# bliunlpr/Robust_e2e_gan

Measured on AMD Instinct MI355X. Metric: joint_train utterances/sec, higher is better.
Workload: dtype f32; 1 GPU; config4: joint_train.py full GAN+ASR step, B=32 per GPU, T=800, F=257->80, L=40, V=4233, enhancer 2xBLSTM-256, VGG+3xBLSTMP-512, loc-attention decoder 300, D basic ndf64, Adadelta; global_batch=32, per_rank_batch=32, parallelism=dp1, utterance_lengths=560..800 frames (mean 680 of T=800)

## Files before the change

robust_e2e_gan_amd/csrc/wino44.hip:

```cpp
#include <hip/hip_runtime.h>
#include "../../include/re2e.h"
#include "common.h"

namespace {

template <class T>
__device__ __forceinline__ void bt5(const T& d0, const T& d1, const T& d2, const T& d3, const T& d4, T (&r)[5]) {
  r[0] = 2.f * d0 - d1 - 2.f * d2 + d3;
  r[1] = -2.f * d1 - d2 + d3;
  r[2] = 2.f * d1 - 3.f * d2 + d3;
  r[3] = d3 - d1;
  r[4] = 2.f * d1 - d2 - 2.f * d3 + d4;
}
__device__ __forceinline__ void g4(float k0, float k1, float k2, float k3, float (&r)[5]) {
  r[0] = 0.5f * k0;
  r[1] = -0.5f * (k0 + k1 + k2 + k3);
  r[2] = (-k0 + k1 - k2 + k3) * (1.f / 6.f);
  r[3] = (k0 + 2.f * k1 + 4.f * k2 + 8.f * k3) * (1.f / 6.f);
  r[4] = k3;
}

__global__ __launch_bounds__(256) void w44_filter_kernel(const float* __restrict__ w, int Cout, int Cin, int dgrad, float* __restrict__ U) {
  const int Cp = dgrad ? Cout : Cin, Op = dgrad ? Cin : Cout;
  const long i = (long)blockIdx.x * 256 + threadIdx.x;
// ... 53 lines not shown
  float* vp = V + p * tile_stride + c4 * 4;
#pragma unroll
  for (int a = 0; a < 5; ++a) {
    f32x4 r[5];
    bt5(t[a][0], t[a][1], t[a][2], t[a][3], t[a][4], r);
#pragma unroll
    for (int b = 0; b < 5; ++b) *reinterpret_cast<f32x4*>(vp + (long)(a * 5 + b) * pos_stride) = r[b];
  }
}

__global__ __launch_bounds__(256) void w44_output_kernel(const float* __restrict__ M, long P, int Cout, int OH, int OW, int ty, int tx,
                                                         float* __restrict__ out) {
  const int o4n = Cout >> 2;
  const long i = (long)blockIdx.x * 256 + threadIdx.x;
  if (i >= P * o4n) return;
  const int o4 = (int)(i % o4n);
  const long p = i / o4n;
  const int x = (int)(p % tx), y = (int)((p / tx) % ty), n = (int)(p / ((long)tx * ty));
  const float* mp = M + p * Cout + o4 * 4;
  const long ps = P * Cout;
  f32x4 s[2][5];
#pragma unroll
  for (int b = 0; b < 5; ++b) {
    f32x4 m[5];
#pragma unroll
    for (int a = 0; a < 5; ++a) m[a] = *reinterpret_cast<const f32x4*>(mp + (long)(a * 5 + b) * ps);
    s[0][b] = m[0] + m[1] + m[2] + m[3];
    s[1][b] = m[1] - m[2] + 2.f * m[3] + m[4];
  }
#pragma unroll
  for (int a = 0; a < 2; ++a) {
    const int oy = 2 * y + a;
    if (oy >= OH) continue;
    const f32x4 y0 = s[a][0] + s[a][1] + s[a][2] + s[a][3];
    const f32x4 y1 = s[a][1] - s[a][2] + 2.f * s[a][3] + s[a][4];
    float* op = out + (((long)n * OH + oy) * OW + 2 * x) * Cout + o4 * 4;
    *reinterpret_cast<f32x4*>(op) = y0;
    if (2 * x + 1 < OW) *reinterpret_cast<f32x4*>(op + Cout) = y1;
  }
}

template <class T>
__device__ __forceinline__ void a5(const T& y0, const T& y1, T (&r)[5]) {
  r[0] = y0; r[1] = y0 + y1; r[2] = y0 - y1; r[3] = y0 + 2.f * y1; r[4] = y1;
}
__global__ __launch_bounds__(256) void w44_dout_kernel(const float* __restrict__ dy, int NI, int OH, int OW, int Cout, int ty, int tx, long P, long Ppad,
                                                       float* __restrict__ dM) {
  const int o4n = Cout >> 2;
  const long i = (long)blockIdx.x * 256 + threadIdx.x;
  if (i >= Ppad * o4n) return;
  const int o4 = (int)(i % o4n);
  const long p = i / o4n;
  const int x = (int)(p % tx), y = (int)((p / tx) % ty), n = p < P ? (int)(p / ((long)tx * ty)) : -1;
  const f32x4 zero = {0.f, 0.f, 0.f, 0.f};
  f32x4 g[2][2];
#pragma unroll
  for (int a = 0; a < 2; ++a)
#pragma unroll
    for (int b = 0; b < 2; ++b) {
      const int oy = 2 * y + a, ox = 2 * x + b;
      g[a][b] = (n >= 0 && oy < OH && ox < OW) ? *reinterpret_cast<const f32x4*>(dy + (((long)n * OH + oy) * OW + ox) * Cout + o4 * 4) : zero;
    }
  f32x4 t0[5], t1[5];
  a5(g[0][0], g[1][0], t0);
  a5(g[0][1], g[1][1], t1);
  float* mp = dM + p * Cout + o4 * 4;
  const long ps = Ppad * Cout;
#pragma unroll
  for (int a = 0; a < 5; ++a) {
    f32x4 r[5];
    a5(t0[a], t1[a], r);
#pragma unroll
    for (int b = 0; b < 5; ++b) *reinterpret_cast<f32x4*>(mp + (long)(a * 5 + b) * ps) = r[b];
  }
}

__global__ __launch_bounds__(256) void w44_wgrad_final_kernel(const float* __restrict__ slabs, int C, int Cout, int sub, float* __restrict__ gw, float beta) {
  const long i = (long)blockIdx.x * 256 + threadIdx.x;
  if (i >= (long)C * Cout) return;
  const int o = (int)(i % Cout), c = (int)(i / Cout);
  const long ss = (long)C * Cout;
  float u[5][5];
#pragma unroll
  for (int pos = 0; pos < 25; ++pos) {
    float v = 0.f;
    for (int z = 0; z < sub; ++z) v += slabs[((long)pos * sub + z) * ss + i];
    u[pos / 5][pos % 5] = v;
  }
  auto gt = [](float v0, float v1, float v2, float v3, float v4, float (&r)[4]) {
    const float s6 = 1.f / 6.f;
    r[0] = 0.5f * v0 - 0.5f * v1 - s6 * v2 + s6 * v3;
    r[1] = -0.5f * v1 + s6 * v2 + 2.f * s6 * v3;
    r[2] = -0.5f * v1 - s6 * v2 + 4.f * s6 * v3;
    r[3] = -0.5f * v1 + s6 * v2 + 8.f * s6 * v3 + v4;
  };
  float t[4][5];
#pragma unroll
  for (int y = 0; y < 5; ++y) {
    float r[4];
    gt(u[0][y], u[1][y], u[2][y], u[3][y], u[4][y], r);
#pragma unroll
    for (int a = 0; a < 4; ++a) t[a][y] = r[a];
  }
  float* wp = gw + ((long)o * C + c) * 16;
#pragma unroll
  for (int a = 0; a < 4; ++a) {
    float r[4];
    gt(t[a][0], t[a][1], t[a][2], t[a][3], t[a][4], r);
#pragma unroll
    for (int b = 0; b < 4; ++b) wp[a * 4 + b] = beta != 0.f ? wp[a * 4 + b] + r[b] : r[b];
  }
}

struct W44Plan { int OH, OW, ty, tx; long P; size_t u_off, v_off, m_off, total; };
W44Plan w44_plan(int NI, int H, int W, int C, int Cout, int pad) {
  W44Plan p;
  p.OH = H + 2 * pad - 3; p.OW = W + 2 * pad - 3;
  p.ty = (p.OH + 1) / 2; p.tx = (p.OW + 1) / 2;
  p.P = (long)NI * p.ty * p.tx;
  auto up = [](size_t b) { return (b + 255) & ~(size_t)255; };
  p.u_off = 0;
  p.v_off = up((size_t)25 * C * Cout * 4);
  p.m_off = p.v_off + up((size_t)p.P * 25 * C * 4);
  p.total = p.m_off + up((size_t)p.P * 25 * Cout * 4);
  return p;
}
}

WinoFit wino4x4_fit(int NI, int H, int W, int C, int Cout, int pad) {
  if (C % 16 || Cout % 4) return kWinoChannels;
  const W44Plan p = w44_plan(NI, H, W, C, Cout, pad);
  return p.P * 25 * C * 4 >= 0xFFFFFFF0L || (long)Cout * 25 * C * 4 >= 0xFFFFFFF0L || p.P >= 0x7fffffffL ? kWinoBytes : kWinoFits;
}

extern "C" size_t re2e_conv4x4_wino_workspace_bytes(int NI, int H, int W, int C, int Cout, int pad) {
  if (NI <= 0 || H <= 0 || W <= 0 || C <= 0 || Cout <= 0 || pad < 0 || H + 2 * pad < 4 || W + 2 * pad < 4) return 0;
  return w44_plan(NI, H, W, C, Cout, pad).total;
}

extern "C" int re2e_conv4x4_wino(const float* in, int NI, int H, int W, int C, const float* w, int Cout, int pad, int dgrad, float* out,
                                 void* workspace, size_t workspace_bytes, hipStream_t stream) {
  RE2E_CHECK_ARG(in && w && out && workspace, "null operand");
  RE2E_CHECK_ARG(NI > 0 && H > 0 && W > 0 && C > 0 && Cout > 0 && pad >= 0 && H + 2 * pad >= 4 && W + 2 * pad >= 4, "bad geometry");
  const WinoFit fit = wino4x4_fit(NI, H, W, C, Cout, pad);
  if (fit == kWinoChannels) { re2e_set_error("re2e_conv4x4_wino: C must be a multiple of 16 and Cout of 4 (got %d, %d)", C, Cout); return RE2E_EUNSUPPORTED; }
  const W44Plan p = w44_plan(NI, H, W, C, Cout, pad);
  RE2E_CHECK_ARG(workspace_bytes >= p.total, "workspace too small (re2e_conv4x4_wino_workspace_bytes)");
  RE2E_CHECK_ARG((reinterpret_cast<uintptr_t>(in) & 15) == 0 && (reinterpret_cast<uintptr_t>(out) & 15) == 0 &&
                 (reinterpret_cast<uintptr_t>(workspace) & 15) == 0, "in / out / workspace must be 16-byte aligned");
  if (fit != kWinoFits) {
    re2e_set_error("re2e_conv4x4_wino: transformed operand larger than 4 GiB");
    return RE2E_EUNSUPPORTED;
  }
  float* U = reinterpret_cast<float*>(static_cast<char*>(workspace) + p.u_off);
  float* V = reinterpret_cast<float*>(static_cast<char*>(workspace) + p.v_off);
  float* M = reinterpret_cast<float*>(static_cast<char*>(workspace) + p.m_off);
  hipLaunchKernelGGL(w44_filter_kernel, dim3((unsigned)cdiv((long)C * Cout, 256)), dim3(256), 0, stream, w, dgrad ? C : Cout, dgrad ? Cout : C, dgrad, U);
  hipLaunchKernelGGL(w44_input_kernel, dim3((unsigned)cdiv(p.P * (C / 4), 256)), dim3(256), 0, stream, in, NI, H, W, C, pad, p.ty, p.tx, V, 25L * C, (long)C, p.P);
  static const bool log_calls = getenv("RE2E_IGEMM_LOG") != nullptr;
  if (log_calls)
    fprintf(stderr, "[igemm] A=W44%s B=DenseK tile=256x128x16 vec=1 M=%ld N=%d K=%d splits=25\n", dgrad ? "D" : "F", (long)NI * p.OH * p.OW, Cout, 16 * C);
  const int rc = gemm_kslices((int)p.P, Cout, 25 * C, 25, V, 25L * C, U, 25L * C, M, stream, 1);
  if (rc != RE2E_OK) return rc;
  hipLaunchKernelGGL(w44_output_kernel, dim3((unsigned)cdiv(p.P * (Cout / 4), 256)), dim3(256), 0, stream, M, p.P, Cout, p.OH, p.OW, p.ty, p.tx, out);
  RE2E_LAUNCH_CHECK();
  return RE2E_OK;
}

namespace {
struct W44WgradPlan { int OH, OW, ty, tx, sub; long P, Ppad; size_t v_off, m_off, s_off, total; };
W44WgradPlan w44_wgrad_plan(int NI, int H, int W, int C, int Cout, int pad) {
  W44WgradPlan p;
  p.OH = H + 2 * pad - 3; p.OW = W + 2 * pad - 3;
  p.ty = (p.OH + 1) / 2; p.tx = (p.OW + 1) / 2;
  p.P = (long)NI * p.ty * p.tx;
  const long tiles = (long)cdiv(C, 128) * cdiv(Cout, 128) * 25;
  int sub = (int)((1024 + tiles - 1) / tiles);
  const long maxsub = p.P / (16 * 64);
  if (sub > maxsub) sub = (int)maxsub;
  if (sub < 1) sub = 1;
  p.sub = sub;
  const long q = 16L * sub;
  p.Ppad = (p.P + q - 1) / q * q;
  auto up = [](size_t b) { return (b + 255) & ~(size_t)255; };
  p.v_off = 0;
  p.m_off = up((size_t)25 * p.Ppad * C * 4);
  p.s_off = p.m_off + up((size_t)25 * p.Ppad * Cout * 4);
  p.total = p.s_off + up((size_t)25 * sub * C * Cout * 4);
  return p;
}
}

WinoFit wino4x4_wgrad_fit(int NI, int H, int W, int C, int Cout, int pad) {
  if (C % 4 || Cout % 4) return kWinoChannels;
  return 25 * w44_wgrad_plan(NI, H, W, C, Cout, pad).Ppad * (long)(C > Cout ? C : Cout) * 4 >= 0xFFFFFFF0L ? kWinoBytes : kWinoFits;
}

extern "C" size_t re2e_conv4x4_wino_wgrad_workspace_bytes(int NI, int H, int W, int C, int Cout, int pad) {
  if (NI <= 0 || H <= 0 || W <= 0 || C <= 0 || Cout <= 0 || pad < 0 || H + 2 * pad < 4 || W + 2 * pad < 4) return 0;
  return w44_wgrad_plan(NI, H, W, C, Cout, pad).total;
}

extern "C" int re2e_conv4x4_wino_wgrad(const float* in, int NI, int H, int W, int C, const float* dout, int Cout, int pad, float* gw, float beta,
                                       void* workspace, size_t workspace_bytes, hipStream_t stream) {
  RE2E_CHECK_ARG(in && dout && gw && workspace, "null operand");
  RE2E_CHECK_ARG(NI > 0 && H > 0 && W > 0 && C > 0 && Cout > 0 && pad >= 0 && H + 2 * pad >= 4 && W + 2 * pad >= 4, "bad geometry");
  RE2E_CHECK_ARG(beta == 0.f || beta == 1.f, "beta must be 0 or 1");
  const WinoFit fit = wino4x4_wgrad_fit(NI, H, W, C, Cout, pad);
  if (fit == kWinoChannels) { re2e_set_error("re2e_conv4x4_wino_wgrad: C and Cout must be multiples of 4 (got %d, %d)", C, Cout); return RE2E_EUNSUPPORTED; }
  const W44WgradPlan p = w44_wgrad_plan(NI, H, W, C, Cout, pad);
  RE2E_CHECK_ARG(workspace_bytes >= p.total, "workspace too small (re2e_conv4x4_wino_wgrad_workspace_bytes)");
  RE2E_CHECK_ARG((reinterpret_cast<uintptr_t>(in) & 15) == 0 && (reinterpret_cast<uintptr_t>(dout) & 15) == 0 &&
                 (reinterpret_cast<uintptr_t>(workspace) & 15) == 0, "in / dout / workspace must be 16-byte aligned");
  if (fit != kWinoFits) { re2e_set_error("re2e_conv4x4_wino_wgrad: transformed operand larger than 4 GiB"); return RE2E_EUNSUPPORTED; }
  float* V = reinterpret_cast<float*>(static_cast<char*>(workspace) + p.v_off);
  float* dM = reinterpret_cast<float*>(static_cast<char*>(workspace) + p.m_off);
  float* S = reinterpret_cast<float*>(static_cast<char*>(workspace) + p.s_off);
  hipLaunchKernelGGL(w44_input_kernel, dim3((unsigned)cdiv(p.Ppad * (C / 4), 256)), dim3(256), 0, stream, in, NI, H, W, C, pad, p.ty, p.tx, V, (long)C,
                     p.Ppad * C, p.Ppad);
  hipLaunchKernelGGL(w44_dout_kernel, dim3((unsigned)cdiv(p.Ppad * (Cout / 4), 256)), dim3(256), 0, stream, dout, NI, p.OH, p.OW, Cout, p.ty, p.tx, p.P,
                     p.Ppad, dM);
  static const bool log_calls = getenv("RE2E_IGEMM_LOG") != nullptr;
  if (log_calls)
    fprintf(stderr, "[igemm] A=W44W B=DenseM tile=128x128x16 vec=1 M=%d N=%d K=%ld splits=%d\n", 16 * C, Cout, (long)NI * p.OH * p.OW, 25 * p.sub);
  const int rc = gemm_kslices_tn(C, Cout, (int)(25 * p.Ppad), 25 * p.sub, V, (long)C, dM, (long)Cout, S, stream, 1);
  if (rc != RE2E_OK) return rc;
  hipLaunchKernelGGL(w44_wgrad_final_kernel, dim3((unsigned)cdiv((long)C * Cout, 256)), dim3(256), 0, stream, S, C, Cout, p.sub, gw, beta);
  RE2E_LAUNCH_CHECK();
  return RE2E_OK;
}
```

robust_e2e_gan_amd/csrc/igemm.hip:

```cpp
#include <stdlib.h>
#include <type_traits>

#include "common.h"

namespace {

template <int WM_, int WN_, int TM_, int TN_, int BK_>
struct Cfg {
  static constexpr int WM = WM_, WN = WN_, TM = TM_, TN = TN_, BK = BK_;
  static constexpr int BM = WM_ * TM_ * 32, BN = WN_ * TN_ * 32;
  static constexpr int THREADS = WM_ * WN_ * 64;
  static constexpr int LDK = BK_ + 4;
};

struct DenseK {
  static constexpr bool KMAJ = true;
  static constexpr const char* NAME = "DenseK";
  static constexpr bool IS_CONVK = false;
  const float* p; unsigned nbytes; long ld; int rows, K;
  struct Row { unsigned base; };
  struct Kst { int k; };
  __device__ void init_row(Row& r, int row) const { r.base = row < rows ? (unsigned)((long)row * ld * 4) : nbytes; }
  __device__ void init_k(Kst& s, int k) const { s.k = k; }
  __device__ void advance(Kst& s, int bk) const { s.k += bk; }
// ... 455 lines not shown
          outp[rb + colv[b]] = sg * mulp[rb + colv[b]];
        }
      }
    return;
  }
  if (ep.beta != 0.f) {
#pragma unroll
    for (int a = 0; a < CF::TM; ++a)
#pragma unroll
      for (int b = 0; b < CF::TN; ++b) {
        float old[16];
        long offs[16];
#pragma unroll
        for (int r = 0; r < 16; ++r) {
          const long rb = row_base(m0 + (wm * CF::TM + a) * 32 + (r & 3) + 8 * (r >> 2) + 4 * lh);
          offs[r] = (rb >= 0 && colv[b] < ep.N) ? rb + colv[b] : -1;
          old[r] = offs[r] >= 0 ? ep.C[offs[r]] : 0.f;
        }
#pragma unroll
        for (int r = 0; r < 16; ++r)
          if (offs[r] >= 0) ep.C[offs[r]] = apply_act(acc[a][b][r] + bv[b], ep.act) + old[r];
      }
    return;
  }
  if (ep.act == RE2E_ACT_TANH || ep.act == RE2E_ACT_SIGMOID) {
    const bool th = ep.act == RE2E_ACT_TANH;
#pragma unroll
    for (int a = 0; a < CF::TM; ++a)
#pragma unroll
      for (int r = 0; r < 16; ++r) {
        const long rb = row_base(m0 + (wm * CF::TM + a) * 32 + (r & 3) + 8 * (r >> 2) + 4 * lh);
        if (rb < 0) continue;
#pragma unroll
        for (int b = 0; b < CF::TN; ++b) {
          const float v = acc[a][b][r] + bv[b];
          if (colv[b] < ep.N) ep.C[rb + colv[b]] = th ? tanhf_(v) : sigmoidf_(v);
        }
      }
    return;
  }
  {
    const float slope = ep.act == RE2E_ACT_RELU ? 0.f : (ep.act == RE2E_ACT_LRELU ? 0.2f : 1.f);
    const bool relu = ep.act == RE2E_ACT_RELU;
#pragma unroll
    for (int a = 0; a < CF::TM; ++a)
#pragma unroll
      for (int r = 0; r < 16; ++r) {
        const long rb = row_base(m0 + (wm * CF::TM + a) * 32 + (r & 3) + 8 * (r >> 2) + 4 * lh);
        if (rb < 0) continue;
#pragma unroll
        for (int b = 0; b < CF::TN; ++b) {
          const float v = acc[a][b][r] + bv[b];
          if (colv[b] < ep.N) ep.C[rb + colv[b]] = v < 0.f ? (relu ? 0.f : slope * v) : v;
        }
      }
  }
}

__global__ void splitk_reduce_kernel(const float* ws, int nsplit, int M, int N, float* C, long ldc, float beta,
                                     int conv_perm, int Cin, int KHW, const float* bias, const float* bias2, int act) {
  long i = (long)blockIdx.x * blockDim.x + threadIdx.x;
  long tot = (long)M * N;
  if (i >= tot) return;
  float s = 0.f;
  for (int z = 0; z < nsplit; ++z) s += ws[(long)z * tot + i];
  int m = (int)(i / N), n = (int)(i % N);
  long off;
  if (conv_perm) { int ci = m % Cin; int tap = m / Cin; off = ((long)n * Cin + ci) * KHW + tap; }
  else off = (long)m * ldc + n;
  if (bias) s += bias[n];
  if (bias2) s += bias2[n];
  s = apply_act(s, act);
  if (beta != 0.f) s += C[off];
  C[off] = s;
}

__global__ __launch_bounds__(1024) void splitk_reduce_wide_kernel(const float* ws, int nsplit, int M, int N, float* C, long ldc,
                                                                  float beta, int conv_perm, int Cin, int KHW) {
  __shared__ float part[16][64];
  const int e = threadIdx.x & 63, sl = threadIdx.x >> 6;
  const long tot = (long)M * N;
  const long i = (long)blockIdx.x * 64 + e;
  float s = 0.f;
  if (i < tot)
    for (int z = sl; z < nsplit; z += 16) s += ws[(long)z * tot + i];
  part[sl][e] = s;
  __syncthreads();
  if (sl != 0 || i >= tot) return;
  s = 0.f;
#pragma unroll
  for (int q = 0; q < 16; ++q) s += part[q][e];
  int m = (int)(i / N), n = (int)(i % N);
  long off;
  if (conv_perm) { int ci = m % Cin; int tap = m / Cin; off = ((long)n * Cin + ci) * KHW + tap; }
  else off = (long)m * ldc + n;
  if (beta != 0.f) s += C[off];
  C[off] = s;
}

template <bool TB, bool VEC>
__global__ __launch_bounds__(512) void skinny_gemm_kernel(const float* __restrict__ A, long lda, const float* __restrict__ B, long ldb,
                                                          float* C, long ldc, int M, int N, int K, const float* __restrict__ bias,
                                                          const float* __restrict__ bias2, float beta) {
  __shared__ float red[8][32][33];
  const int tid = threadIdx.x, lane = tid & 63, wid = tid >> 6, lr = lane & 31, lh = lane >> 5;
  const int n0 = blockIdx.x * 32;
  const int kq = (K + 7) / 8;
  const int per = (kq + 7) / 8;
  const int q0 = wid * per, q1 = min(kq, q0 + per);
  const int row = lr, col = n0 + lr;
  const bool rok = row < M, cok = col < N;
  const float* ap = A + (long)(rok ? row : 0) * lda;
  f32x16 acc;
#pragma unroll
  for (int r = 0; r < 16; ++r) acc[r] = 0.f;
  for (int qb = q0; qb < q1; qb += 4) {
    float av[4][4], bv[4][4];
#pragma unroll
    for (int u = 0; u < 4; ++u) {
      const int k = 8 * (qb + u) + 4 * lh;
      const bool qok = qb + u < q1;
      if (VEC) {
        const bool kok = qok && k < K;
        const f32x4 zero = {0.f, 0.f, 0.f, 0.f};
        const f32x4 a4 = (kok && rok) ? *reinterpret_cast<const f32x4*>(ap + k) : zero;
        f32x4 b4 = zero;
        if (TB) { if (kok && cok) b4 = *reinterpret_cast<const f32x4*>(B + (long)col * ldb + k); }
#pragma unroll
        for (int j = 0; j < 4; ++j) {
          av[u][j] = a4[j];
          bv[u][j] = TB ? b4[j] : ((kok && cok) ? B[(long)(k + j) * ldb + col] : 0.f);
        }
      } else {
#pragma unroll
        for (int j = 0; j < 4; ++j) {
          const bool kok = qok && k + j < K;
          av[u][j] = (kok && rok) ? ap[k + j] : 0.f;
          bv[u][j] = (kok && cok) ? (TB ? B[(long)col * ldb + k + j] : B[(long)(k + j) * ldb + col]) : 0.f;
        }
      }
    }
#pragma unroll
    for (int u = 0; u < 4; ++u)
#pragma unroll
      for (int j = 0; j < 4; ++j) acc = __builtin_amdgcn_mfma_f32_32x32x2f32(av[u][j], bv[u][j], acc, 0, 0, 0);
  }
#pragma unroll
  for (int r = 0; r < 16; ++r) red[wid][(r & 3) + 8 * (r >> 2) + 4 * lh][lr] = acc[r];
  __syncthreads();
  for (int i = tid; i < 32 * 32; i += 512) {
    const int m = i >> 5, n = n0 + (i & 31);
    if (m < M && n < N) {
      float v = 0.f;
#pragma unroll
      for (int w = 0; w < 8; ++w) v += red[w][m][i & 31];
      if (bias) v += bias[n];
      if (bias2) v += bias2[n];
      float* c = C + (long)m * ldc + n;
      *c = (beta != 0.f ? *c : 0.f) + v;
    }
  }
}

__global__ __launch_bounds__(512) void skinny_gemm2_kernel(const float* __restrict__ A, long lda, int M, int K, const float* __restrict__ B1, long ldb1,
                                                           int N1, float* C1, long ldc1, const float* __restrict__ B2, long ldb2, int N2,
                                                           float* C2, long ldc2) {
  __shared__ float red[8][32][33];
  const int tid = threadIdx.x, lane = tid & 63, wid = tid >> 6, lr = lane & 31, lh = lane >> 5;
// ... 775 lines not shown
```

robust_e2e_gan_amd/csrc/wino_wgrad.hip:

```cpp
#include <hip/hip_runtime.h>
#include "../../include/re2e.h"
#include "common.h"

namespace {
typedef float f32x16 __attribute__((ext_vector_type(16)));
typedef float f32x2 __attribute__((ext_vector_type(2)));
constexpr unsigned WW_OOB = 0x80000000u;
constexpr int WW_CB = 64, WW_OB = 32;

struct WwArgs {
  const float* x; const float* dy; float* slabs;
  int NI, H, W, C, Cout;
  int px, py, npatch, nsplit, ncb, nblk;
  unsigned x_bytes, dy_bytes;
  const int* row_lim;
  int flat;
  int dbg;
};

template <int TXW>
__global__ __launch_bounds__(256, 2) void wino_wgrad_kernel(WwArgs p) {
  constexpr int TYH = 32 / TXW, PW = 2 * TXW, PH = 2 * TYH;
  constexpr int XW = PW + 2, XH = PH + 2, XPIX = XW * XH;
  constexpr int XIT = (XPIX * 16 + 255) / 256, DIT = PW * PH * 8 / 256;
// ... 37 lines not shown
  auto store_patch = [&]() {
#pragma unroll
    for (int it = 0; it < XIT; ++it) {
      const int item = it * 256 + tid;
      if (item < XPIX * 16) *reinterpret_cast<f32x4*>(xs + item * 4) = xr[it];
    }
#pragma unroll
    for (int it = 0; it < DIT; ++it) *reinterpret_cast<f32x4*>(ds + (it * 256 + tid) * 4) = dr[it];
  };

  const int rA = wid == 0 ? 0 : (wid == 2 ? 2 : 1), rB = wid == 3 ? 3 : (wid == 2 ? 1 : 2);
  const float sg = wid == 1 ? 1.f : -1.f;
  const float a0 = wid == 3 ? 0.f : 1.f, a1 = wid == 0 ? 0.f : (wid == 1 ? 1.f : -1.f);
  constexpr int HR = TYH / 2;
  const float* xA = xs + ((rA + 2 * HR * lh) * XW) * WW_CB + 2 * lr;
  const float* xB = xs + ((rB + 2 * HR * lh) * XW) * WW_CB + 2 * lr;
  const float* dB = ds + (2 * HR * lh * PW) * WW_OB + lr;

  f32x16 acc[4][2];
#pragma unroll
  for (int j = 0; j < 4; ++j)
#pragma unroll
    for (int ct = 0; ct < 2; ++ct)
#pragma unroll
      for (int r = 0; r < 16; ++r) acc[j][ct][r] = 0.f;

  for (int pi = pbeg; pi < pend; ++pi) {
    if (p.row_lim) {
      const int n = pi / (p.py * p.px), pyi = (pi - n * (p.py * p.px)) / p.px;
      if (pyi * PH >= p.row_lim[n]) continue;
    }
    load_patch(pi);
    store_patch();
    __syncthreads();
    f32x2 t[4], v[2][4];
    float m[2][4];
    auto prep = [&](const int s, f32x2 (&vv)[4], float (&mm)[4]) {
      const int tyl = s / TXW, txl = s % TXW;
#pragma unroll
      for (int j = 0; j < 4; ++j) {
        if (txl != 0 && j < 2) { t[j] = t[j + 2]; continue; }
        const f32x2 da = *reinterpret_cast<const f32x2*>(xA + ((2 * tyl) * XW + 2 * txl + j) * WW_CB);
        const f32x2 db = *reinterpret_cast<const f32x2*>(xB + ((2 * tyl) * XW + 2 * txl + j) * WW_CB);
        t[j] = da + sg * db;
      }
      vv[0] = t[0] - t[2]; vv[1] = t[1] + t[2]; vv[2] = t[2] - t[1]; vv[3] = t[1] - t[3];
      const float e00 = dB[((2 * tyl) * PW + 2 * txl) * WW_OB], e01 = dB[((2 * tyl) * PW + 2 * txl + 1) * WW_OB];
      const float e10 = dB[((2 * tyl + 1) * PW + 2 * txl) * WW_OB], e11 = dB[((2 * tyl + 1) * PW + 2 * txl + 1) * WW_OB];
      const float s0 = a0 * e00 + a1 * e10, s1 = a0 * e01 + a1 * e11;
      mm[0] = s0; mm[1] = s0 + s1; mm[2] = s0 - s1; mm[3] = -s1;
    };
    prep(0, v[0], m[0]);
#pragma unroll
    for (int s = 0; s < 16; ++s) {
      if (s + 1 < 16) prep(s + 1, v[(s + 1) & 1], m[(s + 1) & 1]);
#pragma unroll
      for (int j = 0; j < 4; ++j) {
        acc[j][0] = __builtin_amdgcn_mfma_f32_32x32x2f32(v[s & 1][j][0], m[s & 1][j], acc[j][0], 0, 0, 0);
        acc[j][1] = __builtin_amdgcn_mfma_f32_32x32x2f32(v[s & 1][j][1], m[s & 1][j], acc[j][1], 0, 0, 0);
      }
      if (s + 1 < 16) {
#pragma unroll
        for (int g = 0; g < 8; ++g) {
          __builtin_amdgcn_sched_group_barrier(0x008, 1, 0);
          __builtin_amdgcn_sched_group_barrier(0x100, 1, 0);
          __builtin_amdgcn_sched_group_barrier(0x002, 4, 0);
        }
      }
    }
    __syncthreads();
  }
  float* sl = p.slabs + ((long)split * 16 + 4 * wid) * p.C * p.Cout;
#pragma unroll
  for (int j = 0; j < 4; ++j)
#pragma unroll
    for (int ct = 0; ct < 2; ++ct)
#pragma unroll
      for (int r = 0; r < 16; ++r) {
        const int c = c0 + 2 * ((r & 3) + 8 * (r >> 2) + 4 * lh) + ct;
        sl[((long)j * p.C + c) * p.Cout + o0 + lr] = acc[j][ct][r];
      }
}

__global__ __launch_bounds__(1024) void wino_wgrad_reduce_kernel(const float* __restrict__ slabs, int nsplit, long tot, float* __restrict__ red) {
  __shared__ float part[16][64];
  const int e = threadIdx.x & 63, sl = threadIdx.x >> 6;
  const long i = (long)blockIdx.x * 64 + e;
  float s = 0.f;
  if (i < tot)
    for (int z = sl; z < nsplit; z += 16) s += slabs[(long)z * tot + i];
  part[sl][e] = s;
  __syncthreads();
  if (sl != 0 || i >= tot) return;
  s = 0.f;
#pragma unroll
  for (int q = 0; q < 16; ++q) s += part[q][e];
  red[i] = s;
}

__global__ __launch_bounds__(256) void wino_wgrad_final_kernel(const float* __restrict__ slabs, int nsplit, int C, int Cout, float* __restrict__ gw,
                                                               float beta) {
  const long i = (long)blockIdx.x * 256 + threadIdx.x;
  const long CO = (long)C * Cout;
  if (i >= CO) return;
  const int o = (int)(i % Cout), c = (int)(i / Cout);
  float u[4][4];
#pragma unroll
  for (int pos = 0; pos < 16; ++pos) u[pos >> 2][pos & 3] = 0.f;
  for (int s = 0; s < nsplit; ++s) {
    const float* sp = slabs + (long)s * 16 * CO + i;
#pragma unroll
    for (int pos = 0; pos < 16; ++pos) u[pos >> 2][pos & 3] += sp[pos * CO];
  }
  float t[3][4];
#pragma unroll
  for (int j = 0; j < 4; ++j) {
    t[0][j] = u[0][j] + 0.5f * (u[1][j] + u[2][j]);
    t[1][j] = 0.5f * (u[1][j] - u[2][j]);
    t[2][j] = 0.5f * (u[1][j] + u[2][j]) + u[3][j];
  }
  float* wp = gw + ((long)o * C + c) * 9;
#pragma unroll
  for (int a = 0; a < 3; ++a) {
    const float r0 = t[a][0] + 0.5f * (t[a][1] + t[a][2]), r1 = 0.5f * (t[a][1] - t[a][2]), r2 = 0.5f * (t[a][1] + t[a][2]) + t[a][3];
    if (beta != 0.f) { wp[a * 3] += r0; wp[a * 3 + 1] += r1; wp[a * 3 + 2] += r2; }
    else { wp[a * 3] = r0; wp[a * 3 + 1] = r1; wp[a * 3 + 2] = r2; }
  }
}

struct WwPlan { bool wide; int px, py, npatch, nsplit, ncb, nblk; size_t bytes; };
WwPlan ww_plan(int NI, int H, int W, int C, int Cout) {
  WwPlan q;
  const long pad_w = (long)cdiv(H, 8) * 8 * cdiv(W, 16) * 16, pad_n = (long)cdiv(H, 16) * 16 * cdiv(W, 8) * 8;
  q.wide = pad_w <= pad_n;
  q.px = cdiv(W, q.wide ? 16 : 8); q.py = cdiv(H, q.wide ? 8 : 16);
  q.npatch = NI * q.py * q.px;
  q.ncb = C / WW_CB; q.nblk = q.ncb * (Cout / WW_OB);
  int s = cdiv(1536, q.nblk);
  if (s > q.npatch / 8) s = q.npatch / 8;
  if (s < 1) s = 1;
  q.nsplit = s;
  q.bytes = (size_t)(s + 1) * 16 * C * Cout * sizeof(float);
  return q;
}

template <int TXW>
void launch_ww(const WwArgs& a, hipStream_t st) {
  constexpr int PW = 2 * TXW, PH = 64 / TXW;
  constexpr size_t lds = (size_t)((PW + 2) * (PH + 2) * WW_CB + PW * PH * WW_OB) * sizeof(float);
  static LdsLimit lim;
  lim.ensure(reinterpret_cast<const void*>(&wino_wgrad_kernel<TXW>), lds);
  hipLaunchKernelGGL((wino_wgrad_kernel<TXW>), dim3((unsigned)(cdiv(a.nsplit, 8) * 8 * a.nblk)), dim3(256), lds, st, a);
}
}

extern "C" size_t re2e_conv3x3_wino_wgrad_workspace_bytes(int NI, int H, int W, int C, int Cout) {
  if (NI <= 0 || H <= 0 || W <= 0 || C <= 0 || Cout <= 0 || C % WW_CB || Cout % WW_OB) return 0;
  return ww_plan(NI, H, W, C, Cout).bytes;
}

WinoFit wino3x3_wgrad_fit(int NI, int H, int W, int C, int Cout) {
  if (C % WW_CB || Cout % WW_OB) return kWinoChannels;
  const long x_bytes = (long)NI * H * W * C * 4, dy_bytes = (long)NI * H * W * Cout * 4;
  return x_bytes >= 0x7FFFFF00L || dy_bytes >= 0x7FFFFF00L ? kWinoBytes : kWinoFits;
}

static int ww_impl(const float* in, int NI, int H, int W, int C, const float* dout, int Cout, float* gw, float beta, const int* row_lim, void* workspace,
                   size_t workspace_bytes, hipStream_t stream) {
  RE2E_CHECK_ARG(in && dout && gw && workspace, "null operand");
  RE2E_CHECK_ARG(NI > 0 && H > 0 && W > 0 && C > 0 && Cout > 0, "bad geometry");
  RE2E_CHECK_ARG(beta == 0.f || beta == 1.f, "beta must be 0 or 1");
  const WinoFit fit = wino3x3_wgrad_fit(NI, H, W, C, Cout);
  if (fit == kWinoChannels) { re2e_set_error("re2e_conv3x3_wino_wgrad: C must be a multiple of 64 and Cout of 32 (got %d, %d)", C, Cout); return RE2E_EUNSUPPORTED; }
  if (fit != kWinoFits) { re2e_set_error("re2e_conv3x3_wino_wgrad: tensors must be < 2 GiB"); return RE2E_EUNSUPPORTED; }
  const long x_bytes = (long)NI * H * W * C * 4, dy_bytes = (long)NI * H * W * Cout * 4;
  RE2E_CHECK_ARG((reinterpret_cast<uintptr_t>(in) & 15) == 0 && (reinterpret_cast<uintptr_t>(dout) & 15) == 0, "in / dout must be 16-byte aligned");
  const WwPlan q = ww_plan(NI, H, W, C, Cout);
  RE2E_CHECK_ARG(workspace_bytes >= q.bytes, "workspace too small (re2e_conv3x3_wino_wgrad_workspace_bytes)");
  WwArgs a;
  a.x = in; a.dy = dout; a.slabs = static_cast<float*>(workspace);
  a.NI = NI; a.H = H; a.W = W; a.C = C; a.Cout = Cout;
  a.px = q.px; a.py = q.py; a.npatch = q.npatch; a.nsplit = q.nsplit; a.ncb = q.ncb; a.nblk = q.nblk;
  a.x_bytes = (unsigned)x_bytes; a.dy_bytes = (unsigned)dy_bytes;
  a.row_lim = row_lim;
  a.dbg = exp_env("RE2E_WW_DBG") ? atoi(exp_env("RE2E_WW_DBG")) : 0;
  a.flat = exp_env("RE2E_WW_FLAT") ? atoi(exp_env("RE2E_WW_FLAT")) : 0;
  static const bool log_calls = getenv("RE2E_IGEMM_LOG") != nullptr;
  if (log_calls)
    fprintf(stderr, "[igemm] A=WinoW B=DenseM tile=64x32x2 vec=1 M=%d N=%d K=%ld splits=%d\n", 9 * C, Cout, (long)NI * H * W, q.nsplit);
  if (q.wide) launch_ww<8>(a, stream); else launch_ww<4>(a, stream);
  const long tot = 16L * C * Cout;
  float* red = a.slabs + (long)q.nsplit * tot;
  hipLaunchKernelGGL(wino_wgrad_reduce_kernel, dim3((unsigned)cdiv(tot, 64)), dim3(1024), 0, stream, a.slabs, q.nsplit, tot, red);
  hipLaunchKernelGGL(wino_wgrad_final_kernel, dim3((unsigned)cdiv((long)C * Cout, 256)), dim3(256), 0, stream, red, 1, C, Cout, gw, beta);
  RE2E_LAUNCH_CHECK();
  return RE2E_OK;
}

extern "C" int re2e_conv3x3_wino_wgrad(const float* in, int NI, int H, int W, int C, const float* dout, int Cout, float* gw, float beta, void* workspace,
                                       size_t workspace_bytes, hipStream_t stream) {
  return ww_impl(in, NI, H, W, C, dout, Cout, gw, beta, nullptr, workspace, workspace_bytes, stream);
}

extern "C" int re2e_conv3x3_wino_wgrad_rows(const float* in, int NI, int H, int W, int C, const float* dout, int Cout, float* gw, float beta,
                                            const int* row_lim, void* workspace, size_t workspace_bytes, hipStream_t stream) {
  RE2E_CHECK_ARG(row_lim, "null row limits");
  return ww_impl(in, NI, H, W, C, dout, Cout, gw, beta, row_lim, workspace, workspace_bytes, stream);
}
```

Baseline: 685.8 utterances/s.

## Fuse Winograd 4x4 batched GEMM with output transform in one MFMA kernel

Adds a fused kernel that runs the 25 per-position GEMMs back to back for each output tile, keeping accumulators in registers. After each position it folds the result into the four output-pixel accumulators using the Winograd output-transform coefficients, then writes the final output directly. This removes the intermediate M buffer round trip and the separate output-transform kernel launch. In exchange, GEMM tiles are smaller than the previous 256x128 path and each wave holds extra accumulator registers, which may lower occupancy.

```diff
diff --git a/robust_e2e_gan_amd/csrc/wino44.hip b/robust_e2e_gan_amd/csrc/wino44.hip
--- a/robust_e2e_gan_amd/csrc/wino44.hip
+++ b/robust_e2e_gan_amd/csrc/wino44.hip
@@ -187,6 +187,210 @@
 #pragma unroll
     for (int b = 0; b < 4; ++b) wp[a * 4 + b] = beta != 0.f ? wp[a * 4 + b] + r[b] : r[b];
   }
+}
+
+__constant__ float W44_FOLD[25][4] = {
+    {1, 0, 0, 0}, {1, 1, 0, 0},   {1, -1, 0, 0},  {1, 2, 0, 0},   {0, 1, 0, 0},
+    {1, 0, 1, 0}, {1, 1, 1, 1},   {1, -1, 1, -1}, {1, 2, 1, 2},   {0, 1, 0, 1},
+    {1, 0, -1, 0}, {1, 1, -1, -1}, {1, -1, -1, 1}, {1, 2, -1, -2}, {0, 1, 0, -1},
+    {1, 0, 2, 0}, {1, 1, 2, 2},   {1, -1, 2, -2}, {1, 2, 2, 4},   {0, 1, 0, 2},
+    {0, 0, 1, 0}, {0, 0, 1, 1},   {0, 0, 1, -1},  {0, 0, 1, 2},   {0, 0, 0, 1},
+};
+
+typedef unsigned u32x4_t __attribute__((ext_vector_type(4)));
+constexpr unsigned OOB = 0x80000000u;
+
+template <int WM_, int WN_, int TM_, int TN_, int BK_, int ST_, int WPS_>
+struct W44Cfg {
+  static constexpr int WM = WM_, WN = WN_, TM = TM_, TN = TN_, BK = BK_, ST = ST_, WPS = WPS_;
+  static constexpr int BM = WM_ * TM_ * 32, BN = WN_ * TN_ * 32;
+  static constexpr int NW = WM_ * WN_, THREADS = NW * 64;
+  static constexpr int RPP = 256 / BK, CPR = BK / 4, RPL = 64 / BK;
+  static constexpr int PA = BM / RPP, PB = BN / RPP;
+  static constexpr int NPW = (PA + PB) / NW, NPA = PA / NW;
+  static constexpr int STAGE = (BM + BN) * BK;
+  static constexpr int NQ = BK / 8;
+  static constexpr size_t LDS_BYTES = (size_t)ST_ * STAGE * 4;
+  static_assert(BK_ == 16 || BK_ == 32, "BK");
+  static_assert(PA % NW == 0 && PB % NW == 0, "pieces must divide over the waves per operand");
+  static_assert((ST_ - 1) * NPW < 64, "vmcnt is a 6-bit counter");
+};
+using W44x128x64w8 = W44Cfg<4, 2, 1, 1, 32, 3, 4>;
+using W44x128x64 = W44Cfg<2, 2, 2, 1, 16, 4, 2>;
+constexpr int W44_FUSED_DEFAULT = 1;
+
+struct W44FusedArgs {
+  const float* V; const float* U; float* out;
+  unsigned v_bytes, u_bytes, out_bytes;
+  int ld;
+  int P, Cout, nkt;
+  int OH, OW, ty, tx, ntm, ntn;
+};
+
+template <int N>
+__device__ __forceinline__ void wait_vmcnt() { asm volatile("s_waitcnt vmcnt(%0)" ::"n"(N) : "memory"); }
+__device__ __forceinline__ void wait_lgkm0() { asm volatile("s_waitcnt lgkmcnt(0)" ::: "memory"); }
+__device__ __forceinline__ void wg_barrier() {
+  asm volatile("" ::: "memory");
+  __builtin_amdgcn_s_barrier();
+  asm volatile("" ::: "memory");
+}
+__device__ __forceinline__ int xcd_chunk(int orig, int n) {
+  const int q8 = n >> 3, r8 = n & 7, xcd = orig & 7;
+  return (xcd < r8 ? xcd * (q8 + 1) : r8 * (q8 + 1) + (xcd - r8) * q8) + (orig >> 3);
+}
+
+template <class CF>
+__global__ __launch_bounds__(CF::THREADS, CF::WPS) void w44_fused_kernel(W44FusedArgs p) {
+  constexpr int BM = CF::BM, BN = CF::BN, BK = CF::BK, ST = CF::ST, TM = CF::TM, TN = CF::TN, NW = CF::NW;
+  constexpr int NPW = CF::NPW, NPA = CF::NPA, NQ = CF::NQ, STAGE = CF::STAGE, CPR = CF::CPR, RPL = CF::RPL, RPP = CF::RPP;
+  extern __shared__ __attribute__((aligned(1024))) float smem[];
+  const int tid = threadIdx.x, lane = tid & 63;
+  const int wid = __builtin_amdgcn_readfirstlane(tid >> 6);
+  const int wm = wid / CF::WN, wn = wid % CF::WN;
+  const int lr = lane & 31, lh = lane >> 5;
+  const __amdgpu_buffer_rsrc_t rsV = __builtin_amdgcn_make_buffer_rsrc(const_cast<float*>(p.V), 0, p.v_bytes, 0x00020000);
+  const __amdgpu_buffer_rsrc_t rsU = __builtin_amdgcn_make_buffer_rsrc(const_cast<float*>(p.U), 0, p.u_bytes, 0x00020000);
+
+  const int tile = xcd_chunk((int)blockIdx.x, p.ntm * p.ntn);
+  const int tile_m = tile / p.ntn, tile_n = tile - tile_m * p.ntn;
+  const int m0 = tile_m * BM, n0 = tile_n * BN;
+
+  const int prow = lane / CPR, cpos = lane % CPR;
+  unsigned voff[NPW];
+#pragma unroll
+  for (int i = 0; i < NPW; ++i) {
+    const bool isA = i < NPA;
+    const int prow_t = ((isA ? i : i - NPA) * NW + wid) * RPP + prow;
+    const unsigned pc16 = (unsigned)((cpos ^ ((prow_t / RPL) % CPR)) * 16);
+    const int row = (isA ? m0 : n0) + prow_t;
+    voff[i] = row < (isA ? p.P : p.Cout) ? (unsigned)row * (unsigned)p.ld * 4u + pc16 : OOB;
+  }
+  const int xs = lh ^ ((lr / RPL) % CPR);
+  const int a_row0 = wm * TM * 32 + lr, b_row0 = wn * TN * 32 + lr;
+  const int nkt = p.nkt, nkt_all = 25 * nkt;
+
+  auto issue = [&](int slot, int kt) {
+    const bool dead = kt >= nkt_all;
+    const unsigned soff = dead ? 0u : (unsigned)kt * (unsigned)(BK * 4);
+    float* base = smem + slot * STAGE + wid * 256;
+#pragma unroll
+    for (int i = 0; i < NPW; ++i) {
+      const unsigned v = dead ? OOB : voff[i];
+      __builtin_amdgcn_raw_ptr_buffer_load_lds(i < NPA ? rsV : rsU, (__attribute__((address_space(3))) void*)(base + i * NW * 256), 16, v, soff, 0, 0);
+    }
+  };
+
+  f32x16 acc[TM][TN], y[4][TM][TN];
+#pragma unroll
+  for (int a = 0; a < TM; ++a)
+#pragma unroll
+    for (int b = 0; b < TN; ++b)
+#pragma unroll
+      for (int r = 0; r < 16; ++r) {
+        acc[a][b][r] = 0.f;
+#pragma unroll
+        for (int j = 0; j < 4; ++j) y[j][a][b][r] = 0.f;
+      }
+
+  f32x4 fa[2][TM], fb[2][TN];
+  auto read_frags = [&](int slot, int q, int buf) {
+    const float* S = smem + slot * STAGE;
+    const int co = ((2 * q) ^ xs) << 2;
+#pragma unroll
+    for (int a = 0; a < TM; ++a) fa[buf][a] = *reinterpret_cast<const f32x4*>(S + (a_row0 + a * 32) * BK + co);
+#pragma unroll
+    for (int b = 0; b < TN; ++b) fb[buf][b] = *reinterpret_cast<const f32x4*>(S + BM * BK + (b_row0 + b * 32) * BK + co);
+  };
+  auto mfma_group = [&](int buf) {
+#pragma unroll
+    for (int j = 0; j < 4; ++j)
+#pragma unroll
+      for (int a = 0; a < TM; ++a)
+#pragma unroll
+        for (int b = 0; b < TN; ++b) acc[a][b] = __builtin_amdgcn_mfma_f32_32x32x2f32(fb[buf][b][j], fa[buf][a][j], acc[a][b], 0, 0, 0);
+  };
+
+#pragma unroll
+  for (int s = 0; s < ST; ++s) issue(s, s);
+  wait_vmcnt<(ST - 1) * NPW>();
+  wg_barrier();
+  read_frags(0, 0, 0);
+  int slot = 0, ktg = 0;
+#pragma unroll 1
+  for (int pos = 0; pos < 25; ++pos) {
+#pragma unroll 1
+    for (int kt = 0; kt < nkt; ++kt, ++ktg) {
+      const int nslot = slot + 1 == ST ? 0 : slot + 1;
+#pragma unroll
+      for (int q = 0; q < NQ - 1; ++q) {
+        read_frags(slot, q + 1, (q + 1) & 1);
+        mfma_group(q & 1);
+      }
+      wait_lgkm0();
+      wait_vmcnt<(ST - 2) * NPW>();
+      wg_barrier();
+      issue(slot, ktg + ST);
+      read_frags(nslot, 0, NQ & 1);
+      mfma_group((NQ - 1) & 1);
+      slot = nslot;
+    }
+#pragma unroll
+    for (int j = 0; j < 4; ++j) {
+      const float c = W44_FOLD[pos][j];
+      if (c != 0.f) {
+#pragma unroll
+        for (int a = 0; a < TM; ++a)
+#pragma unroll
+          for (int b = 0; b < TN; ++b)
+#pragma unroll
+            for (int r = 0; r < 16; ++r) y[j][a][b][r] = fmaf(c, acc[a][b][r], y[j][a][b][r]);
+      }
+    }
+#pragma unroll
+    for (int a = 0; a < TM; ++a)
+#pragma unroll
+      for (int b = 0; b < TN; ++b)
+#pragma unroll
+        for (int r = 0; r < 16; ++r) acc[a][b][r] = 0.f;
+  }
+  wait_vmcnt<0>();
+
+  const __amdgpu_buffer_rsrc_t rsO = __builtin_amdgcn_make_buffer_rsrc(p.out, 0, p.out_bytes, 0x00020000);
+  unsigned vrow[TM][4];
+#pragma unroll
+  for (int a = 0; a < TM; ++a) {
+    const int t = m0 + (wm * TM + a) * 32 + lr;
+    const int x = t % p.tx, t2 = t / p.tx, yy = t2 % p.ty, n = t2 / p.ty;
+#pragma unroll
+    for (int j = 0; j < 4; ++j) {
+      const int oy = 2 * yy + (j >> 1), ox = 2 * x + (j & 1);
+      const bool ok = t < p.P && oy < p.OH && ox < p.OW;
+      vrow[a][j] = ok ? (unsigned)(((((long)n * p.OH + oy) * p.OW + ox) * p.Cout + 4 * lh) * 4) : OOB;
+    }
+  }
+#pragma unroll
+  for (int j = 0; j < 4; ++j)
+#pragma unroll
+    for (int b = 0; b < TN; ++b)
+#pragma unroll
+      for (int g = 0; g < 4; ++g) {
+        const int colq = n0 + (wn * TN + b) * 32 + 8 * g;
+        const bool col_ok = colq + 4 * lh < p.Cout;
+#pragma unroll
+        for (int a = 0; a < TM; ++a) {
+          const unsigned vo = (col_ok && vrow[a][j] != OOB) ? vrow[a][j] + (unsigned)colq * 4u : OOB;
+          const f32x4 v = {y[j][a][b][4 * g], y[j][a][b][4 * g + 1], y[j][a][b][4 * g + 2], y[j][a][b][4 * g + 3]};
+          __builtin_amdgcn_raw_buffer_store_b128(__builtin_bit_cast(u32x4_t, v), rsO, vo, 0, 0);
+        }
+      }
+}
+
+template <class CF>
+void w44_fused_launch(const W44FusedArgs& a, hipStream_t st) {
+  static LdsLimit lim;
+  lim.ensure(reinterpret_cast<const void*>(&w44_fused_kernel<CF>), CF::LDS_BYTES);
+  hipLaunchKernelGGL((w44_fused_kernel<CF>), dim3((unsigned)(a.ntm * a.ntn)), dim3(CF::THREADS), CF::LDS_BYTES, st, a);
 }
 
 struct W44Plan { int OH, OW, ty, tx; long P; size_t u_off, v_off, m_off, total; };
@@ -235,6 +439,24 @@
   hipLaunchKernelGGL(w44_filter_kernel, dim3((unsigned)cdiv((long)C * Cout, 256)), dim3(256), 0, stream, w, dgrad ? C : Cout, dgrad ? Cout : C, dgrad, U);
   hipLaunchKernelGGL(w44_input_kernel, dim3((unsigned)cdiv(p.P * (C / 4), 256)), dim3(256), 0, stream, in, NI, H, W, C, pad, p.ty, p.tx, V, 25L * C, (long)C, p.P);
   static const bool log_calls = getenv("RE2E_IGEMM_LOG") != nullptr;
+  const char* fe = getenv("RE2E_W44_FUSED");
+  int fused = fe ? atoi(fe) : W44_FUSED_DEFAULT;
+  const long out_bytes = (long)NI * p.OH * p.OW * Cout * 4;
+  if (p.P * 25 * C * 4 >= 0x7FFFFFF0L || (long)Cout * 25 * C * 4 >= 0x7FFFFFF0L || out_bytes >= 0x7FFFFFF0L) fused = 0;
+  if (fused == 1 && C % 32) fused = 2;
+  if (fused == 1 || fused == 2) {
+    const int bm = 128, bn = 64, bk = fused == 1 ? 32 : 16;
+    if (log_calls)
+      fprintf(stderr, "[igemm] A=W44%s B=DenseK tile=%dx%dx%d vec=1 M=%ld N=%d K=%d splits=25\n", dgrad ? "D" : "F", bm, bn, bk, (long)NI * p.OH * p.OW, Cout, 16 * C);
+    W44FusedArgs a;
+    a.V = V; a.U = U; a.out = out;
+    a.v_bytes = (unsigned)(p.P * 25 * C * 4); a.u_bytes = (unsigned)((long)Cout * 25 * C * 4); a.out_bytes = (unsigned)out_bytes;
+    a.ld = 25 * C; a.P = (int)p.P; a.Cout = Cout; a.nkt = C / bk;
+    a.OH = p.OH; a.OW = p.OW; a.ty = p.ty; a.tx = p.tx; a.ntm = cdiv(p.P, bm); a.ntn = cdiv(Cout, bn);
+    if (fused == 1) w44_fused_launch<W44x128x64w8>(a, stream); else w44_fused_launch<W44x128x64>(a, stream);
+    RE2E_LAUNCH_CHECK();
+    return RE2E_OK;
+  }
   if (log_calls)
     fprintf(stderr, "[igemm] A=W44%s B=DenseK tile=256x128x16 vec=1 M=%ld N=%d K=%d splits=25\n", dgrad ? "D" : "F", (long)NI * p.OH * p.OW, Cout, 16 * C);
   const int rc = gemm_kslices((int)p.P, Cout, 25 * C, 25, V, 25L * C, U, 25L * C, M, stream, 1);
```

Result: no change. 688.4 utterances/s, median of 6 (+0.4%).

## Fuse Winograd wgrad split reduction with final transform; batch loads in reductions

Applied to the files above, without the earlier changes.

The separate split-K reduce kernel and the Winograd filter-transform kernel are merged into one finish kernel. It loads slabs with 128-bit buffer loads, several splits in flight per thread, reduces in shared memory, then applies the output transform, so the intermediate reduced buffer and one launch go away. The igemm split-K wide reduce and the 4x4 Winograd wgrad final kernel also batch their independent loads ahead of the accumulation to raise memory-level parallelism. This adds a guard that rejects slabs at or above 2 GiB, and it assumes C*Cout is a multiple of 32.

```diff
diff --git a/robust_e2e_gan_amd/csrc/igemm.hip b/robust_e2e_gan_amd/csrc/igemm.hip
--- a/robust_e2e_gan_amd/csrc/igemm.hip
+++ b/robust_e2e_gan_amd/csrc/igemm.hip
@@ -561,8 +561,17 @@
   const long tot = (long)M * N;
   const long i = (long)blockIdx.x * 64 + e;
   float s = 0.f;
-  if (i < tot)
-    for (int z = sl; z < nsplit; z += 16) s += ws[(long)z * tot + i];
+  if (i < tot) {
+    int z = sl;
+    for (; z + 7 * 16 < nsplit; z += 8 * 16) {
+      float v[8];
+#pragma unroll
+      for (int k = 0; k < 8; ++k) v[k] = ws[(long)(z + 16 * k) * tot + i];
+#pragma unroll
+      for (int k = 0; k < 8; ++k) s += v[k];
+    }
+    for (; z < nsplit; z += 16) s += ws[(long)z * tot + i];
+  }
   part[sl][e] = s;
   __syncthreads();
   if (sl != 0 || i >= tot) return;
diff --git a/robust_e2e_gan_amd/csrc/wino44.hip b/robust_e2e_gan_amd/csrc/wino44.hip
--- a/robust_e2e_gan_amd/csrc/wino44.hip
+++ b/robust_e2e_gan_amd/csrc/wino44.hip
@@ -159,10 +159,13 @@
   const long ss = (long)C * Cout;
   float u[5][5];
 #pragma unroll
-  for (int pos = 0; pos < 25; ++pos) {
-    float v = 0.f;
-    for (int z = 0; z < sub; ++z) v += slabs[((long)pos * sub + z) * ss + i];
-    u[pos / 5][pos % 5] = v;
+  for (int pos = 0; pos < 25; ++pos) u[pos / 5][pos % 5] = 0.f;
+  for (int z = 0; z < sub; ++z) {
+    float v[25];
+#pragma unroll
+    for (int pos = 0; pos < 25; ++pos) v[pos] = slabs[((long)pos * sub + z) * ss + i];
+#pragma unroll
+    for (int pos = 0; pos < 25; ++pos) u[pos / 5][pos % 5] += v[pos];
   }
   auto gt = [](float v0, float v1, float v2, float v3, float v4, float (&r)[4]) {
     const float s6 = 1.f / 6.f;
diff --git a/robust_e2e_gan_amd/csrc/wino_wgrad.hip b/robust_e2e_gan_amd/csrc/wino_wgrad.hip
--- a/robust_e2e_gan_amd/csrc/wino_wgrad.hip
+++ b/robust_e2e_gan_amd/csrc/wino_wgrad.hip
@@ -143,36 +143,50 @@
       }
 }
 
-__global__ __launch_bounds__(1024) void wino_wgrad_reduce_kernel(const float* __restrict__ slabs, int nsplit, long tot, float* __restrict__ red) {
-  __shared__ float part[16][64];
-  const int e = threadIdx.x & 63, sl = threadIdx.x >> 6;
-  const long i = (long)blockIdx.x * 64 + e;
-  float s = 0.f;
-  if (i < tot)
-    for (int z = sl; z < nsplit; z += 16) s += slabs[(long)z * tot + i];
-  part[sl][e] = s;
+__global__ __launch_bounds__(1024) void wino_wgrad_finish_kernel(const float* __restrict__ slabs, unsigned slab_bytes, int nsplit, int C, int Cout,
+                                                                 float* __restrict__ gw, float beta) {
+  constexpr int E = 32, L4 = E / 4, PG = 64 / L4, PPT = 16 / PG, ZB = 16 / PPT;
+  __shared__ __attribute__((aligned(16))) float part[16][16][E];
+  __shared__ float us[16][E];
+  const int tid = threadIdx.x, l4 = tid % L4, q = (tid / L4) & 15, pg = tid / (L4 * 16);
+  const unsigned CO = (unsigned)C * Cout, i0 = blockIdx.x * E;
+  const __amdgpu_buffer_rsrc_t rs = __builtin_amdgcn_make_buffer_rsrc(const_cast<float*>(slabs), 0, slab_bytes, 0x00020000);
+  f32x4 s[PPT];
+#pragma unroll
+  for (int pp = 0; pp < PPT; ++pp) s[pp] = f32x4{0.f, 0.f, 0.f, 0.f};
+  for (int z0 = q; z0 < nsplit; z0 += 16 * ZB) {
+    f32x4 v[ZB][PPT];
+#pragma unroll
+    for (int k = 0; k < ZB; ++k)
+#pragma unroll
+      for (int pp = 0; pp < PPT; ++pp) {
+        const int z = z0 + 16 * k;
+        const unsigned off = ((((unsigned)z * 16 + pg * PPT + pp) * CO) + i0 + l4 * 4) * 4;
+        v[k][pp] = __builtin_bit_cast(f32x4, __builtin_amdgcn_raw_buffer_load_b128(rs, z < nsplit ? off : WW_OOB, 0, 0));
+      }
+    __builtin_amdgcn_sched_barrier(0);
+#pragma unroll
+    for (int k = 0; k < ZB; ++k)
+#pragma unroll
+      for (int pp = 0; pp < PPT; ++pp) s[pp] += v[k][pp];
+  }
+#pragma unroll
+  for (int pp = 0; pp < PPT; ++pp) *reinterpret_cast<f32x4*>(&part[q][pg * PPT + pp][l4 * 4]) = s[pp];
   __syncthreads();
-  if (sl != 0 || i >= tot) return;
-  s = 0.f;
-#pragma unroll
-  for (int q = 0; q < 16; ++q) s += part[q][e];
-  red[i] = s;
-}
-
-__global__ __launch_bounds__(256) void wino_wgrad_final_kernel(const float* __restrict__ slabs, int nsplit, int C, int Cout, float* __restrict__ gw,
-                                                               float beta) {
-  const long i = (long)blockIdx.x * 256 + threadIdx.x;
-  const long CO = (long)C * Cout;
-  if (i >= CO) return;
+  if (tid < 16 * E) {
+    const int pos = tid / E, e = tid % E;
+    float t = 0.f;
+#pragma unroll
+    for (int qq = 0; qq < 16; ++qq) t += part[qq][pos][e];
+    us[pos][e] = t;
+  }
+  __syncthreads();
+  if (tid >= E) return;
+  const unsigned i = i0 + tid;
   const int o = (int)(i % Cout), c = (int)(i / Cout);
   float u[4][4];
 #pragma unroll
-  for (int pos = 0; pos < 16; ++pos) u[pos >> 2][pos & 3] = 0.f;
-  for (int s = 0; s < nsplit; ++s) {
-    const float* sp = slabs + (long)s * 16 * CO + i;
-#pragma unroll
-    for (int pos = 0; pos < 16; ++pos) u[pos >> 2][pos & 3] += sp[pos * CO];
-  }
+  for (int pos = 0; pos < 16; ++pos) u[pos >> 2][pos & 3] = us[pos][tid];
   float t[3][4];
 #pragma unroll
   for (int j = 0; j < 4; ++j) {
@@ -238,6 +252,7 @@
   RE2E_CHECK_ARG((reinterpret_cast<uintptr_t>(in) & 15) == 0 && (reinterpret_cast<uintptr_t>(dout) & 15) == 0, "in / dout must be 16-byte aligned");
   const WwPlan q = ww_plan(NI, H, W, C, Cout);
   RE2E_CHECK_ARG(workspace_bytes >= q.bytes, "workspace too small (re2e_conv3x3_wino_wgrad_workspace_bytes)");
+  if (q.bytes >= 0x7FFFFF00UL) { re2e_set_error("re2e_conv3x3_wino_wgrad: C * Cout too large (the slabs must stay under 2 GiB)"); return RE2E_EUNSUPPORTED; }
   WwArgs a;
   a.x = in; a.dy = dout; a.slabs = static_cast<float*>(workspace);
   a.NI = NI; a.H = H; a.W = W; a.C = C; a.Cout = Cout;
@@ -250,10 +265,9 @@
   if (log_calls)
     fprintf(stderr, "[igemm] A=WinoW B=DenseM tile=64x32x2 vec=1 M=%d N=%d K=%ld splits=%d\n", 9 * C, Cout, (long)NI * H * W, q.nsplit);
   if (q.wide) launch_ww<8>(a, stream); else launch_ww<4>(a, stream);
-  const long tot = 16L * C * Cout;
-  float* red = a.slabs + (long)q.nsplit * tot;
-  hipLaunchKernelGGL(wino_wgrad_reduce_kernel, dim3((unsigned)cdiv(tot, 64)), dim3(1024), 0, stream, a.slabs, q.nsplit, tot, red);
-  hipLaunchKernelGGL(wino_wgrad_final_kernel, dim3((unsigned)cdiv((long)C * Cout, 256)), dim3(256), 0, stream, red, 1, C, Cout, gw, beta);
+  const long CO = (long)C * Cout;
+  const unsigned slab_bytes = (unsigned)((size_t)q.nsplit * 16 * CO * sizeof(float));
+  hipLaunchKernelGGL(wino_wgrad_finish_kernel, dim3((unsigned)(CO / 32)), dim3(1024), 0, stream, a.slabs, slab_bytes, q.nsplit, C, Cout, gw, beta);
   RE2E_LAUNCH_CHECK();
   return RE2E_OK;
 }
```

Result: no change. 690.8 utterances/s before, 689.9 utterances/s after (-0.1%).
